# ronen-halevy/yolo-v3-tf2

Hardware: AMD Instinct MI355X
Metric: images/sec at 416x416 batch=64, f32 (full YOLOv3 detect: conv stack + decode + NMS) (higher is better)
Workload: dtype f32

## Files before the change

include/y3.h:

```cpp
#ifndef Y3_H
#define Y3_H

#include <stddef.h>
#include <stdint.h>

#ifdef __cplusplus
extern "C" {
#endif

typedef int y3_status;
enum {
    Y3_OK = 0,
    Y3_ERR_INVALID = -1,
    Y3_ERR_HIP = -2,
    Y3_ERR_OOM = -3,
    Y3_ERR_STATE = -4,
    Y3_ERR_NODEVICE = -5,
    Y3_ERR_COMM = -6,
    Y3_ERR_INTERNAL = -7
};

enum { Y3_DTYPE_F32 = 0, Y3_DTYPE_BF16 = 1, Y3_DTYPE_F32X3 = 2, Y3_DTYPE_F32X2 = 3, Y3_DTYPE_F16 = 4, Y3_DTYPE_I8 = 5 };

int y3_version(void);
// ... 22 lines not shown

enum { Y3_AUX_ADD = 0, Y3_AUX_UPSAMPLE2X = 1, Y3_AUX_CONCAT = 2 };
typedef struct {
    int32_t kind;
    int32_t src0;
    int32_t src1;
    int32_t dst;
} y3_aux_desc;

typedef struct {
    int32_t channels;
    int32_t div;
} y3_tensor_desc;

y3_status y3_net_create(const y3_tensor_desc *tensors, int n_tensors, const int32_t *op_kinds, int n_ops,
                        const y3_conv_desc *convs, int n_convs, const y3_aux_desc *aux, int n_aux,
                        int input_tensor, const int32_t outputs[3], int nclasses, y3_net **out);
void y3_net_destroy(y3_net *net);

y3_status y3_net_set_conv_weights(y3_net *net, int conv_slot, const float *w, const float *gamma,
                                  const float *beta, const float *mean, const float *var, const float *bias,
                                  float eps);

y3_status y3_net_set_tile(y3_net *net, int conv_slot, int tile);
y3_status y3_net_set_tile_bf16(y3_net *net, int conv_slot, int tile);
y3_status y3_net_set_tile_x3(y3_net *net, int conv_slot, int tile);
y3_status y3_net_set_tile_x2(y3_net *net, int conv_slot, int tile);
y3_status y3_net_set_lanes(y3_net *net, int lanes);
y3_status y3_net_set_xcd_mode(y3_net *net, int mode);
y3_status y3_net_set_k_chunk(y3_net *net, int channels);
y3_status y3_net_set_border_skip(y3_net *net, int mode);
int y3_net_get_border_skip(const y3_net *net, int conv_slot, int batch);
void y3_border_order(int Ho, int Wo, int H, int W, int stride, int pad, uint32_t *out);
y3_status y3_net_set_low_latency(y3_net *net, int on);
y3_status y3_net_set_split_k(y3_net *net, int conv_slot, int S);
int y3_net_get_split_k(const y3_net *net, int conv_slot);
int y3_choose_split_k(long long tiles, int k_tiles, int n_cus, long long slab_bytes_per_slice);
y3_status y3_net_set_low_latency_bf16(y3_net *net, int on);
y3_status y3_net_set_split_k_bf16(y3_net *net, int conv_slot, int S);
int y3_net_get_split_k_bf16(const y3_net *net, int conv_slot);
y3_status y3_net_set_low_latency_f16(y3_net *net, int on);
y3_status y3_net_set_split_k_f16(y3_net *net, int conv_slot, int S);
int y3_net_get_split_k_f16(const y3_net *net, int conv_slot);
y3_status y3_net_keep_activations(y3_net *net, int keep);
y3_status y3_net_set_stem_fusion(y3_net *net, int on);
y3_status y3_net_set_stem_fusion_f16(y3_net *net, int on);
y3_status y3_net_measure_sclk(y3_net *net, const float *images_dev, int batch, float *const grids_dev[3], int forwards,
                              float *mhz_out, void *stream);
y3_status y3_net_measure_sclk_conv(y3_net *net, const float *images_dev, int batch, float *const grids_dev[3], int forwards,
                                   int conv, float *mhz_out, void *stream);
y3_status y3_net_measure_sclk_all(y3_net *net, const float *images_dev, int batch, float *const grids_dev[3], int forwards,
                                  float *mhz_out, double *start_us, double *end_us, void *stream);
y3_status y3_net_set_early_chunk(y3_net *net, int n_convs, int chunk_images);

y3_status y3_net_plan(y3_net *net, int max_batch, int image_size, int dtype);

y3_status y3_net_plan_hw(y3_net *net, int max_batch, int height, int width, int dtype);

y3_status y3_net_forward(y3_net *net, const float *images_dev, int batch, float *const grids_dev[3], void *stream);

y3_status y3_net_read_tensor(y3_net *net, int tensor_id, int batch, float *dst_dev, size_t *n_elems, void *stream);

y3_status y3_net_set_act_scales(y3_net *net, const float *scales, int n_tensors);
float y3_net_get_act_scale(const y3_net *net, int tensor_id);
int y3_net_i8_first_conv(const y3_net *net);
y3_status y3_net_read_tensor_i8(y3_net *net, int tensor_id, int batch, int8_t *dst_dev, size_t *n_elems, void *stream);
// ... 89 lines not shown
```

yolo-v3-tf2_amd/_lib.py:

```python
from __future__ import annotations

import ctypes as C
import os

from . import PACKAGE_DIR

LIB_PATH = os.environ.get("Y3_LIB_PATH") or os.path.join(PACKAGE_DIR, "lib", "liby3hip.so")

Y3_OK = 0
Y3_DTYPE_F32, Y3_DTYPE_BF16, Y3_DTYPE_F32X3, Y3_DTYPE_F32X2, Y3_DTYPE_F16, Y3_DTYPE_I8 = 0, 1, 2, 3, 4, 5
DTYPE_TAGS = {Y3_DTYPE_F32: "f32", Y3_DTYPE_BF16: "bf16", Y3_DTYPE_F32X3: "f32x3", Y3_DTYPE_F32X2: "f32x2", Y3_DTYPE_F16: "f16", Y3_DTYPE_I8: "i8"}
TILES_I8_BUILT = (8, 10, 11, 12, 17, 19, 24, 26, 27, 29)
TILES_X2_BUILT = (0, 1, 2, 3, 4, 8, 12, 26, 27)
TILES_X3_BUILT = (0, 1, 2, 3, 4, 8, 9, 12, 13, 14)
Y3_AUX_ADD, Y3_AUX_UPSAMPLE2X, Y3_AUX_CONCAT = 0, 1, 2
_Z = (0, 0, 0, 0)
TILES = [_Z, _Z, _Z, _Z, _Z, _Z,
         (128, 128, 4, 1), _Z, (256, 32, 4, 1), (128, 64, 4, 1), (64, 128, 4, 1), (64, 64, 4, 1),
         (128, 128, 8, 1), _Z, _Z, _Z,
         _Z, (128, 64, 8, 1), _Z, _Z,
         _Z, _Z, _Z,
         (128, 128, 4, 1), _Z,
         _Z,
         (64, 128, 4, 2), (64, 64, 4, 2), _Z, _Z, _Z,
# ... 42 lines not shown
class TensorDesc(C.Structure):
    _fields_ = [("channels", C.c_int32), ("div", C.c_int32)]


class ImageDesc(C.Structure):
    _fields_ = [("offset", C.c_uint64), ("height", C.c_int32), ("width", C.c_int32), ("channels", C.c_int32),
                ("mode", C.c_int32)]


_vp, _i, _f, _sz = C.c_void_p, C.c_int, C.c_float, C.c_size_t
_fp = C.POINTER(C.c_float)

SYMBOLS = {
    "y3_version": (_i, []),
    "y3_last_error": (C.c_char_p, []),
    "y3_device_count": (_i, []),
    "y3_tile_built": (_i, [_i, _i]),
    "y3_net_create": (_i, [C.POINTER(TensorDesc), _i, C.POINTER(C.c_int32), _i, C.POINTER(ConvDesc), _i,
                           C.POINTER(AuxDesc), _i, _i, C.POINTER(C.c_int32), _i, C.POINTER(_vp)]),
    "y3_net_destroy": (None, [_vp]),
    "y3_net_set_conv_weights": (_i, [_vp, _i, _fp, _fp, _fp, _fp, _fp, _fp, _f]),
    "y3_net_set_tile": (_i, [_vp, _i, _i]),
    "y3_net_set_tile_bf16": (_i, [_vp, _i, _i]),
    "y3_net_set_tile_x3": (_i, [_vp, _i, _i]),
    "y3_net_set_tile_x2": (_i, [_vp, _i, _i]),
    "y3_net_set_early_chunk": (_i, [_vp, _i, _i]),
    "y3_net_keep_activations": (_i, [_vp, _i]),
    "y3_net_set_lanes": (_i, [_vp, _i]),
    "y3_net_set_xcd_mode": (_i, [_vp, _i]),
    "y3_net_set_k_chunk": (_i, [_vp, _i]),
    "y3_net_set_border_skip": (_i, [_vp, _i]),
    "y3_net_get_border_skip": (_i, [_vp, _i, _i]),
    "y3_border_order": (None, [_i, _i, _i, _i, _i, _i, C.POINTER(C.c_uint32)]),
    "y3_net_set_stem_fusion": (_i, [_vp, _i]),
    "y3_net_set_low_latency": (_i, [_vp, _i]),
    "y3_net_set_split_k": (_i, [_vp, _i, _i]),
    "y3_net_get_split_k": (_i, [_vp, _i]),
    "y3_choose_split_k": (_i, [C.c_longlong, _i, _i, C.c_longlong]),
    "y3_net_set_low_latency_bf16": (_i, [_vp, _i]),
    "y3_net_set_split_k_bf16": (_i, [_vp, _i, _i]),
    "y3_net_get_split_k_bf16": (_i, [_vp, _i]),
    "y3_net_set_low_latency_f16": (_i, [_vp, _i]),
    "y3_net_set_split_k_f16": (_i, [_vp, _i, _i]),
    "y3_net_get_split_k_f16": (_i, [_vp, _i]),
    "y3_net_set_stem_fusion_f16": (_i, [_vp, _i]),
    "y3_net_measure_sclk": (_i, [_vp, _vp, _i, C.POINTER(_vp), _i, _fp, _vp]),
    "y3_net_measure_sclk_conv": (_i, [_vp, _vp, _i, C.POINTER(_vp), _i, _i, _fp, _vp]),
    "y3_net_measure_sclk_all": (_i, [_vp, _vp, _i, C.POINTER(_vp), _i, _fp, C.POINTER(C.c_double), C.POINTER(C.c_double), _vp]),
    "y3_net_plan": (_i, [_vp, _i, _i, _i]),
    "y3_net_plan_hw": (_i, [_vp, _i, _i, _i, _i]),
    "y3_net_forward": (_i, [_vp, _vp, _i, C.POINTER(_vp), _vp]),
    "y3_net_read_tensor": (_i, [_vp, _i, _i, _vp, C.POINTER(_sz), _vp]),
    "y3_net_set_act_scales": (_i, [_vp, _fp, _i]),
    "y3_net_get_act_scale": (_f, [_vp, _i]),
    "y3_net_i8_first_conv": (_i, [_vp]),
    "y3_net_read_tensor_i8": (_i, [_vp, _i, _i, _vp, C.POINTER(_sz), _vp]),
    "y3_net_flops_per_image": (C.c_double, [_vp]),
    "y3_net_profile_convs": (_i, [_vp, _vp, _i, _fp, _i, _vp]),
    "y3_preprocess_image": (_i, [_vp, _i, _i, _i, _i, _vp, _i, _i, _vp]),
    "y3_preprocess_image_hw": (_i, [_vp, _i, _i, _i, _i, _vp, _i, _i, _i, _vp]),
    "y3_preprocess_batch": (_i, [_vp, _sz, C.POINTER(ImageDesc), _i, _vp, _i, _i, _vp]),
    "y3_preprocess_batch_hw": (_i, [_vp, _sz, C.POINTER(ImageDesc), _i, _vp, _i, _i, _i, _vp]),
    "y3_letterbox_geometry": (_i, [C.POINTER(ImageDesc), _i, _i, C.POINTER(C.c_int32)]),
    "y3_letterbox_geometry_hw": (_i, [C.POINTER(ImageDesc), _i, _i, _i, C.POINTER(C.c_int32)]),
    "y3_unletterbox_detections": (_i, [_vp, _vp, C.POINTER(C.c_int32), _i, _i, _i, _vp]),
    "y3_unletterbox_detections_hw": (_i, [_vp, _vp, C.POINTER(C.c_int32), _i, _i, _i, _i, _vp]),
# ... 74 lines not shown
```

yolo-v3-tf2_amd/csrc/conv_f32.hip:

```cpp
#include <algorithm>
#include <type_traits>

#include "conv_common.h"

namespace y3 {

static constexpr int BK = 32;
static constexpr int lds_row(int dma) { return dma ? BK : BK + 4; }

__device__ __forceinline__ f32x4 buf_load16(__amdgpu_buffer_rsrc_t r, unsigned voff, int soff)
{
    u32x4 v = __builtin_amdgcn_raw_buffer_load_b128(r, (int)voff, soff, 0);
    return __builtin_bit_cast(f32x4, v);
}

#ifdef Y3_PHASE_STAMPS
__device__ unsigned long long y3_dbg32_stamps[8 * 32768];
__device__ int y3_dbg32_sel_k = -1;
#define Y3_STAMP32(k) do { if (threadIdx.x == 0 && blockIdx.x < 32768 && p.K == y3_dbg32_sel_k) y3_dbg32_stamps[blockIdx.x * 8 + (k)] = __builtin_amdgcn_s_memrealtime(); } while (0)
#else
#define Y3_STAMP32(k) do { } while (0)
#endif

template <int TM, int TN, int WR, int WC, bool CONCAT, int STAGES, int MINW = 1, int DMA = 0, bool SPLIT = false, bool BMIN = false>
// ... 12 lines not shown
    constexpr int LDS_ROW = lds_row(DMA);
    constexpr int BM = 32 * TM * WR;
    constexpr int BN = 32 * TN * WC;
    constexpr int NT = 64 * WR * WC;
    constexpr int RP = NT / 8;
    constexpr int AP = BM / RP;
    constexpr int BP = BN / RP;
    static_assert(BM % RP == 0 && BN % RP == 0 && AP >= 1 && BP >= 1, "tile too small for the thread count");
    constexpr int STAGE = (BM + BN) * LDS_ROW;
    extern __shared__ __attribute__((aligned(16))) float smem[];

    const int tid = threadIdx.x;
    if constexpr (!SPLIT) clk_stamp_entry(p.clk_stamps);
    const int lane = tid & 63;
    const int wave = __builtin_amdgcn_readfirstlane(tid >> 6);
    const int wr = wave / WC, wc = wave % WC;

    const int nwg = gridDim.x;
    const int bid = blockIdx.x, xcd = bid & 7;
    const int logical = xcd_contiguous_tile(bid, nwg);
    const int tilesN = p.CoutPad / BN;
    const int kt0 = SPLIT ? (int)blockIdx.y * (p.K / BK) / (int)gridDim.y : 0;
    int KT = SPLIT ? ((int)blockIdx.y + 1) * (p.K / BK) / (int)gridDim.y - kt0 : p.K / BK;
    const __amdgpu_buffer_rsrc_t rs0 = buffer_rsrc(p.src0, p.src0_bytes);
    const __amdgpu_buffer_rsrc_t rs1 = buffer_rsrc(CONCAT ? p.src1 : p.src0, CONCAT ? p.src1_bytes : p.src0_bytes);
    const __amdgpu_buffer_rsrc_t rsw = buffer_rsrc(p.wpk, p.w_bytes);
    const unsigned OOB0 = p.src0_bytes, OOB1 = CONCAT ? p.src1_bytes : p.src0_bytes;

    const __amdgpu_buffer_rsrc_t rsd = buffer_rsrc(p.dst, p.dst_bytes);
    const __amdgpu_buffer_rsrc_t rsr = buffer_rsrc(p.residual ? p.residual : p.dst, p.dst_bytes);
    const int fr = lane & 31, fh = lane >> 5;

    int mt = logical / tilesN, nt = logical - mt * tilesN;
    if (p.xcd_gn > 0) {
        const int gn = p.xcd_gn, gm = 8 / gn;
        const int tilesM = (p.M + BM - 1) / BM;
        const int xm = xcd / gn, xn = xcd - xm * gn;
        const int nb = tilesN / gn;
        const int mlo = xm * tilesM / gm, mhi = (xm + 1) * tilesM / gm;
        const int j = bid >> 3;
        const int lm = j / nb;
        mt = mlo + lm;
        nt = xn * nb + (j - lm * nb);
        if (mt >= mhi) return;
    }
    const int m0 = mt * BM, n0 = nt * BN;

    const int lrow = tid >> 3;
    const int lchunk = DMA ? swizzled_chunk<8>(lrow, tid & 7) * 4 : (tid & 7) * 4;
    int aoff[AP];
    int aoff1[CONCAT ? AP : 1];
    int ahw[AP];
    const int C1 = p.Cin - p.C0;
    constexpr int NBLK = BMIN ? BM / 32 : 1;
    TileBlocks blk{0, 0, 1, 0x1ffu};
    unsigned eent[BMIN ? TM : 1];
    int eimg[BMIN ? TM : 1];
    if constexpr (BMIN) {
        blk = tile_blocks<NBLK>(p, m0);
        if (blk.live == 0) blk.live = 1;
        KT = __builtin_popcount(blk.live) * (p.Cin / BK);
#pragma unroll
        for (int i = 0; i < TM; ++i) tile_block<NBLK>(p, blk, wr * TM + i, eent[i], eimg[i]);
    } else {
        const TileOrigin org = tile_origin(p, m0);
#pragma unroll
        for (int i = 0; i < AP; ++i)
// ... 308 lines not shown
    const int m = (int)(idx / per_row);
    const int n = ((int)(idx - (size_t)m * per_row)) * W;
    const float *src = ws + (size_t)m * cout_pad + n;
    vec v = *reinterpret_cast<const vec *>(src);
    for (int s = 1; s < S; ++s) v = v + *reinterpret_cast<const vec *>(src + (size_t)s * slab_elems);
    v = v + *reinterpret_cast<const vec *>(shift + n);
    if (leaky) {
        const vec t = v * 0.1f;
#pragma unroll
        for (int k = 0; k < W; ++k) v[k] = fmaxf(v[k], t[k]);
    }
    const size_t o = (size_t)m * cout + n;
    if (residual) v = *reinterpret_cast<const vec *>(residual + o) + v;
    *reinterpret_cast<vec *>(dst + o) = v;
}

template <int TM, int TN, int WR, int WC, bool CONCAT, int STAGES, int MINW, int DMA>
static hipError_t launch_k(const ConvArgs &a, hipStream_t s)
{
    constexpr int BM = 32 * TM * WR, BN = 32 * TN * WC;
    const int tilesM = (a.M + BM - 1) / BM, tilesN = a.CoutPad / BN;
    const size_t lds = STAGES * (size_t)(BM + BN) * lds_row(DMA) * sizeof(float);
    int grid = tilesM * tilesN;
    if (a.xcd_gn > 0) {
        if (8 % a.xcd_gn || tilesN % a.xcd_gn) return hipErrorInvalidValue;
        const int gm = 8 / a.xcd_gn;
        int rows = 0;
        for (int xm = 0; xm < gm; ++xm) rows = std::max(rows, (xm + 1) * tilesM / gm - xm * tilesM / gm);
        grid = 8 * rows * (tilesN / a.xcd_gn);
    }
    if constexpr (!CONCAT) {
        if (a.pos_tab) {
            if (a.ksize != 3 || a.B < 32 || a.B % 32 || a.M != a.B * a.Ho * a.Wo || a.Ho > kPosMaxGrid || a.Wo > kPosMaxGrid) return hipErrorInvalidValue;
            return launch_conv_kernel<conv_f32_mfma<TM, TN, WR, WC, false, STAGES, MINW, DMA, false, true>>(a, grid, 64 * WR * WC, lds, s);
        }
    } else if (a.pos_tab) {
        return hipErrorInvalidValue;
    }
    return launch_conv_kernel<conv_f32_mfma<TM, TN, WR, WC, CONCAT, STAGES, MINW, DMA>>(a, grid, 64 * WR * WC, lds, s);
}

template <int TM, int TN, int WR, int WC, int STAGES, int MINW, int DMA>
static hipError_t launch_t(const ConvArgs &a, hipStream_t s)
{
    return a.src1 ? launch_k<TM, TN, WR, WC, true, STAGES, MINW, DMA>(a, s) : launch_k<TM, TN, WR, WC, false, STAGES, MINW, DMA>(a, s);
}

struct TileF32 { TileInfo info; hipError_t (*launch)(const ConvArgs &, hipStream_t); };
template <int TM, int TN, int WR, int WC, int STAGES = 1, int MINW = 1, int DMA = 0>
static constexpr TileF32 tile() { return {{32 * TM * WR, 32 * TN * WC, WR * WC, STAGES, BK}, launch_t<TM, TN, WR, WC, STAGES, MINW, DMA>}; }

static hipError_t launch_res(const ConvArgs &a, hipStream_t s) { return conv_res_f32_fits(a) ? launch_conv_res_f32(a, s) : hipErrorInvalidValue; }

static const TileF32 kTiles[TILE_COUNT] = {
    {}, {}, {}, {}, {}, {},
    tile<2, 2, 2, 2>(),
    {},
    tile<2, 1, 4, 1>(),
    tile<1, 2, 4, 1, 1, 4>(),
    tile<1, 2, 2, 2, 1, 4>(),
    tile<1, 1, 2, 2, 1, 4>(),
    tile<2, 1, 2, 4>(),
    {}, {}, {}, {},
    tile<1, 1, 4, 2>(),
    {}, {}, {}, {}, {},
    tile<2, 2, 2, 2, 1, 3>(),
// ... 57 lines not shown
```

yolo-v3-tf2_amd/csrc/y3_forward.cpp:

```cpp
#include <cstdlib>
#include <vector>

#include "y3_host.h"

struct Forward {
    const float *images;
    float *const *grids;
    int batch;
    hipStream_t stream;
    int lanes;
    const y3::DecodeHead *heads = nullptr;
    unsigned long long *clk = nullptr;
    int clk_conv = -1;
    float *ms_out = nullptr;
    int n_ms = 0;
};

static y3_status check_forward_args(const y3_net *net, bool args_ok, int batch, bool heads, const char *who)
{
    if (!net || !args_ok || batch <= 0) return fail(Y3_ERR_INVALID, "%s: bad argument", who);
    if (heads && net->nclasses <= 0) return fail(Y3_ERR_STATE, "%s: the net was created without detection heads (nclasses = 0)", who);
    if (!net->height) return fail(Y3_ERR_STATE, "%s: call y3_net_plan first", who);
    if (batch > net->max_batch) return fail(Y3_ERR_INVALID, "%s: batch %d > planned %d", who, batch, net->max_batch);
    return Y3_OK;
// ... 159 lines not shown
        if (x.kind == Y3_AUX_ADD)
            e = y3::launch_add(p(x.src0), p(x.src1), p(x.dst), (size_t)nb * sh * sw * C, s);
        else if (x.kind == Y3_AUX_UPSAMPLE2X)
            e = y3::launch_upsample2x(p(x.src0), nb, sh / 2, sw / 2, C, p(x.dst), s);
        else if (x.kind == Y3_AUX_CONCAT)
            e = y3::launch_concat(p(x.src0), net->tensors[x.src0].channels, p(x.src1), net->tensors[x.src1].channels, (size_t)nb * sh * sw, p(x.dst), s);
        else
            return fail(Y3_ERR_INVALID, "unknown aux op kind %d", x.kind);
        if (e != hipSuccess) return fail(Y3_ERR_HIP, "aux op %d launch: %s", index, hipGetErrorString(e));
        return Y3_OK;
    }

    y3_status run(int op_begin, int op_end) const
    {
        hipEvent_t ev0 = nullptr, ev1 = nullptr;
        if (f.ms_out) {
            HIP_TRY(hipEventCreate(&ev0));
            HIP_TRY(hipEventCreate(&ev1));
        }
        if (op_begin == 0 && crosses(net->input_tensor))
            if (y3_status st = quantize_crossing(net->input_tensor); st != Y3_OK) return st;
        for (int oi = op_begin; oi < op_end; ++oi) {
            const Op &o = net->ops[oi];
            if (o.kind != 0) {
                if (y3_status st = run_aux(o.index); st != Y3_OK) return st;
                continue;
            }
            y3::ConvArgs a = conv_args(o.index);
            if (!a.src0 || (!a.dst && !a.dec.boxes)) return fail(Y3_ERR_STATE, "conv %d: tensor not planned", o.index);
            const y3::ConvChoice ch = y3::choose_conv(net, oi, a);
            a.k_chunk = ch.k_chunk;
            a.xcd_gn = ch.xcd_gn;
            a.pos_tab = ch.pos_tab;
            if (ch.kind == y3::ConvKind::InStem) {
                if (f.ms_out && o.index < f.n_ms) f.ms_out[o.index] = 0.0f;
            } else {
                if (f.ms_out) HIP_TRY(hipEventRecord(ev0, s));
                if (y3_status st = launch_conv(oi, a, ch); st != Y3_OK) return st;
                if (f.ms_out) {
                    HIP_TRY(hipEventRecord(ev1, s));
                    HIP_TRY(hipEventSynchronize(ev1));
                    float ms = 0;
                    HIP_TRY(hipEventElapsedTime(&ms, ev0, ev1));
                    if (o.index < f.n_ms) f.ms_out[o.index] = ms;
                }
            }
            const int dst = net->convs[o.index].d.dst;
            if (crosses(dst))
                if (y3_status st = quantize_crossing(dst); st != Y3_OK) return st;
        }
        for (int k = 0; k < 3 && op_end == (int)net->ops.size(); ++k) {
            const int t = net->outputs[k];
            if (!net->staged[t]) continue;
            const size_t npix = (size_t)nb * rows(net, t) * cols(net, t);
            float *out = f.grids[k] + (size_t)b0 * img_elems(t);
            hipError_t e = net->dtype != Y3_DTYPE_I8 ? y3::launch_to_f32(net->dtype, ptr(t), out, npix, net->tensors[t].channels, s)
                           : net->telem[t] == 1      ? y3::launch_i8_to_f32(ptr(t), out, npix * net->tensors[t].channels, net->tscale[t], s)
                                                     : y3::launch_to_f32(Y3_DTYPE_F16, ptr(t), out, npix, net->tensors[t].channels, s);
            if (e != hipSuccess) return fail(Y3_ERR_HIP, "output %d conversion: %s", k, hipGetErrorString(e));
        }
        if (f.ms_out) {
            (void)hipEventDestroy(ev0);
            (void)hipEventDestroy(ev1);
        }
        return Y3_OK;
    }
// ... 320 lines not shown
```

yolo-v3-tf2_amd/csrc/y3_host.h:

```cpp
#pragma once
#include <hip/hip_runtime.h>

#include <vector>

#include "../../include/y3.h"
#include "y3_kernels.h"

namespace y3 {
int fail_msg(int code, const char *fmt, ...) noexcept;
int on_exception(const char *who) noexcept;
bool test_fail_alloc() noexcept;
}

#define Y3_CATCH(who) catch (...) { return y3::on_exception(who); }

constexpr auto fail = y3::fail_msg;

#define HIP_TRY(expr)                                                                             \
    do {                                                                                          \
        hipError_t e_ = (expr);                                                                   \
        if (e_ != hipSuccess)                                                                     \
            return fail(e_ == hipErrorOutOfMemory ? Y3_ERR_OOM : Y3_ERR_HIP, "%s: %s", #expr,     \
                        hipGetErrorString(e_));                                                   \
    } while (0)
// ... 17 lines not shown
struct ConvSlot {
    y3_conv_desc d{};
    bool loaded = false;
    bool first_layer = false;
    int cout_pad = 0;
    int K = 0;
    int tile = -1;
    int split_req = -1;
    int split_req_bf16 = -1;
    int split_req_f16 = -1;
    int split_k = 1;
    int tile_bf16 = -1;
    int tile_x3 = -1;
    int cout_pad64 = 0;
    void *wx3_dev = nullptr;
    int tile_x2 = -1;
    bool x2_ok = true;
    void *wx2_dev = nullptr;
    float *scale_x2_dev = nullptr;
    void *w_dev = nullptr;
    float *w0stem_dev = nullptr;
    float *w0raw_dev = nullptr;
    float *w0norm_dev = nullptr;
    float *scale0norm_dev = nullptr;
    void *wbf_dev = nullptr;
    void *wf16_dev = nullptr;
    float *scale_dev = nullptr;
    float *shift_dev = nullptr;
    void *wi8_dev = nullptr;
    std::vector<float> sw_host, bn_scale_host;
    float *sc_i8_dev = nullptr;
    float q_res = 0.0f, q_inv = 0.0f;
    const uint32_t *pos_tab = nullptr;
};

struct Op {
    int kind;
    int index;
};

constexpr int Y3_MAX_LANES = 4;
constexpr int Y3_MAX_OUTPUT_BOXES = 1024;

struct y3_net {
    int device = 0;
    int n_cus = 0;
    std::vector<y3_tensor_desc> tensors;
    std::vector<Op> ops;
    std::vector<ConvSlot> convs;
    std::vector<y3_aux_desc> aux;
    int input_tensor = 0;
    int outputs[3] = {0, 0, 0};
    int nclasses = 0;
    int max_batch = 0, height = 0, width = 0, dtype = Y3_DTYPE_F32;
    int keep_all = 0;
    int lanes = 1;
    int early_convs = 0;
    int early_chunk = 0;
    int early_ops = 0;
    std::vector<char> dense;
    std::vector<char> staged;
    std::vector<signed char> out_slot;
    void *det_buf = nullptr;
    size_t det_bytes = 0;
    int stem_mode = 1;
    bool stem_mode_set = false;
    int stem_mode_f16 = 0;
    bool stem_fused = false;
    bool stem_conv2 = false;
    int xcd_mode = 1;
    bool low_latency_set = false;
    bool low_latency = false;
    bool low_latency_bf16 = false;
    bool low_latency_f16 = false;
    void *split_ws = nullptr;
    size_t split_ws_lane = 0;
    int split_ws_lanes = 0;
    int k_chunk = -1;
    int border_skip = -1;
    struct PosTab { int Ho, Wo, H, W, stride; uint32_t *dev; };
    std::vector<PosTab> pos_tabs;
    hipEvent_t fork_ev = nullptr;
    hipStream_t lane_stream[4] = {nullptr, nullptr, nullptr, nullptr};
    hipEvent_t join_ev[4] = {nullptr, nullptr, nullptr, nullptr};
    std::vector<void *> tdev;
    std::vector<size_t> tbytes;
    std::vector<size_t> tblock;
    std::vector<void *> blocks;
    std::vector<float> act_scale;
    int i8_first_conv = -1;
    std::vector<unsigned char> telem;
    std::vector<char> tcross;
    std::vector<void *> tq8;
    std::vector<float> tscale;
};

inline int rows(const y3_net *n, int t) { return n->height / n->tensors[t].div; }
inline int cols(const y3_net *n, int t) { return n->width / n->tensors[t].div; }
inline bool is_output(const y3_net *net, int t) { return t == net->outputs[0] || t == net->outputs[1] || t == net->outputs[2]; }

namespace y3 {

struct ConvChoice;
struct SplitForm {
    bool (*tile)(int);
    hipError_t (*launch)(const ConvArgs &, int tile, bool out_f32, int S, void *ws, size_t ws_bytes, hipStream_t);
    int bk, min_k_tiles;
    int ConvSlot::*req;
    bool y3_net::*low_latency;
    const char *set_split, *set_switch;
    const char *(*no_form)(int tile);
    const char *tiles, *other_plan;
    int cout_mult;
// ... 3 lines not shown
    int count;
    TileInfo (*info)(int);
    bool (*built)(int);
    int ConvSlot::*tile;
    int ConvSlot::*cout_pad;
    const char *bad, *retired, *misfit;
    int resident;
    y3_status (*resident_rule)(const y3_net *, const ConvSlot &, int slot);
    void *ConvSlot::*w;
    int elem_bytes;
    int (*choose)(const ConvSlot &, long long M, long long M_plan, bool arena_out);
    hipError_t (*launch)(const ConvArgs &, int tile, bool out_f32, hipStream_t);
    void (*refine)(const y3_net *, const ConvSlot &, const ConvArgs &, ConvChoice &);
    hipError_t (*launch_stem)(const StemArgs &, hipStream_t);
    float *ConvSlot::*w0_stem;
    float *ConvSlot::*scale0_stem;
    int y3_net::*stem_mode;
    const SplitForm *split;
};
const ConvFamily *conv_family(int dtype);
inline const ConvFamily &family_of(const y3_net *net) { return *conv_family(net->dtype); }
inline bool conv_is_i8(const y3_net *net, int slot) { return net->dtype == Y3_DTYPE_I8 && net->i8_first_conv >= 0 && slot >= net->i8_first_conv; }
inline int dtype_of_conv(const y3_net *net, int slot) { return net->dtype != Y3_DTYPE_I8 || conv_is_i8(net, slot) ? net->dtype : (int)Y3_DTYPE_F16; }
inline const ConvFamily &family_of_conv(const y3_net *net, int slot) { return *conv_family(dtype_of_conv(net, slot)); }

enum class ConvKind { First, Stem, InStem, HeadDecodeF32, Mfma, SplitK };
struct ConvChoice {
    ConvKind kind;
    int tile;
    int k_chunk;
    int xcd_gn;
    int split_k;
    const uint32_t *pos_tab;
};
ConvChoice choose_conv(const y3_net *net, int oi, const ConvArgs &a);
ConvChoice choose_conv_planned(const y3_net *net, int oi);
int conv_op(const y3_net *net, int slot);

bool stem_applicable(const y3_net *net);
bool stem_conv2_applicable(const y3_net *net);
void resolve_stem(y3_net *net);
bool output_staged(const y3_net *net, int t);
y3_status resolve_splits(y3_net *net);
y3_status resolve_border(y3_net *net);
y3_status resolve_i8(y3_net *net);
y3_status upload_i8_scales(y3_net *net, int slot);
void free_plan(y3_net *net);

struct DetectLayout {
    int32_t gs[3][2];
    size_t n_boxes;
    size_t grid[3], boxes, cls, scores, sel, nms_ws, total;
};
DetectLayout detect_layout(const y3_net *net, int batch);

y3_status decode_scores_hw(const char *who, const float *const grids_dev[3], const int32_t (*grid_hw)[2], int batch, int nclasses,
                           const float *anchors_host, float *bboxes_dev, int64_t *class_idx_dev, float *scores_dev, void *stream);

}
```

yolo-v3-tf2_amd/csrc/y3_kernels.h:

```cpp
#pragma once
#include <hip/hip_runtime.h>
#include <stddef.h>
#include <stdint.h>
#include <type_traits>

#include "../../include/y3.h"
#include "decode_box.h"

namespace y3 {

struct ConvArgs {
    const void *src0;
    const void *src1;
    const void *wpk;
    const float *scale;
    const float *shift;
    const void *residual;
    void *dst;
    int B, H, W;
    int Ho, Wo;
    int Cin, C0;
    int Cout, CoutPad;
    int ksize, stride, pad;
    int up0;
    int leaky;
    int M;
    int K;
    unsigned src0_bytes, src1_bytes, w_bytes, dst_bytes;
    int xcd_gn;
    DecodeHead dec;
    int k_chunk;
    unsigned long long *clk_stamps;
    int n_cus;
    int device;
    float q_res, q_inv;
    const uint32_t *pos_tab;
};

constexpr int kPosMaxGrid = 2047;
constexpr int kPosTabPad = 8;
constexpr uint32_t pos_pack(int ho, int wo, uint32_t mask9) { return ((uint32_t)ho << 20) | ((uint32_t)wo << 9) | mask9; }
constexpr int pos_ho(uint32_t e) { return (int)(e >> 20); }
constexpr int pos_wo(uint32_t e) { return (int)((e >> 9) & 0x7ffu); }
constexpr uint32_t pos_mask(uint32_t e) { return e & 0x1ffu; }
void border_order(int Ho, int Wo, int H, int W, int stride, int pad, uint32_t *out);

struct LdsAttrOnce { unsigned long long done = 0; };
inline hipError_t set_max_lds_once(LdsAttrOnce &st, const void *fn, int bytes, int dev = -1)
{
    hipError_t e = hipSuccess;
    if (dev < 0 && (e = hipGetDevice(&dev)) != hipSuccess) return e;
    if (dev >= 0 && dev < 64 && ((st.done >> dev) & 1ull)) return hipSuccess;
    e = hipFuncSetAttribute(fn, hipFuncAttributeMaxDynamicSharedMemorySize, bytes);
    if (e == hipSuccess && dev >= 0 && dev < 64) st.done |= 1ull << dev;
    return e;
}

template <auto KERNEL>
static hipError_t launch_conv_kernel(const ConvArgs &a, int grid, int threads, size_t lds, hipStream_t s, int grid_y = 1)
{
    if (lds > 160 * 1024) return hipErrorInvalidValue;
    static LdsAttrOnce attr;
    if (hipError_t e = set_max_lds_once(attr, reinterpret_cast<const void *>(KERNEL), (int)lds, a.device); e != hipSuccess) return e;
    hipLaunchKernelGGL(KERNEL, dim3(grid, grid_y), dim3(threads), lds, s, a);
    return hipGetLastError();
}

template <typename LAUNCH>
static hipError_t dispatch_concat_out(bool concat, bool out_f32, LAUNCH launch)
{
// ... 152 lines not shown
```

yolo-v3-tf2_amd/csrc/y3_net.cpp:

```cpp
#include <algorithm>
#include <cmath>
#include <cstdarg>
#include <cstdio>
#include <cstdlib>
#include <cstring>
#include <exception>
#include <memory>
#include <new>

#include "y3_host.h"

namespace {

thread_local char g_err[512] = "";

}

namespace y3 {
int fail_msg(int code, const char *fmt, ...) noexcept
{
    va_list ap;
    va_start(ap, fmt);
    vsnprintf(g_err, sizeof(g_err), fmt, ap);
    va_end(ap);
// ... 202 lines not shown
        return blocks(27) >= 512 ? 27 : 29;
    }
    if (bf16_out && c.d.size == 3 && c.d.stride == 1 && c.d.src1 < 0 && (c.d.cin == 32 || c.d.cin == 64) && c.d.cout % 64 == 0) return 32;
    static constexpr int bk32[] = {5, 6},
                         n128[] = {8, 12, 11},
                         n64[] = {10, 11}, n32[] = {4};
    if (c.d.cin % 64) return first_reaching(bk32, y3::conv_bf16_tile_info, c, c.cout_pad, M, 512);
    if (c.cout_pad % 128 == 0) return first_reaching(n128, y3::conv_bf16_tile_info, c, c.cout_pad, M, 512);
    if (c.cout_pad % 64 == 0) return first_reaching(n64, y3::conv_bf16_tile_info, c, c.cout_pad, M, 512);
    return first_reaching(n32, y3::conv_bf16_tile_info, c, c.cout_pad, M, 512);
}

int choose_tile_i8(const ConvSlot &c, long long M, long long M_plan, bool arena_out)
{
    const int t = choose_tile_bf16(c, M, M_plan, arena_out);
    if (y3::conv_i8_tile_built(t) && fits(y3::conv_i8_tile_info(t), c, c.cout_pad64)) return t;
    static constexpr int n64[] = {10, 11};
    return first_reaching(n64, y3::conv_i8_tile_info, c, c.cout_pad64, M, 512);
}

int default_k_chunk(const ConvSlot &c)
{
    static const int env = [] { const char *e = getenv("Y3_K_CHUNK"); return e ? atoi(e) : -1; }();
    if (env >= 0) return env;
    return (c.d.size == 3 && c.d.cin >= 256) ? 128 : 0;
}

constexpr int kBorderSkipMaxPositions = 1 << 30;
bool default_border_skip(const y3::ConvArgs &a)
{
    static const int env = [] { const char *e = getenv("Y3_BORDER_SKIP"); return e ? atoi(e) : -1; }();
    static const int max_pos = [] { const char *e = getenv("Y3_BORDER_SKIP_MAX_POS"); return e ? atoi(e) : kBorderSkipMaxPositions; }();
    return env != 0 && a.Ho * a.Wo <= max_pos;
}

int choose_xcd_gn(const ConvSlot &c, const y3::ConvArgs &a, const y3::TileInfo &t)
{
    const int tilesN = a.CoutPad / t.bn;
    const long long tilesM = (a.M + t.bm - 1) / t.bm;
    if (tilesM * tilesN < 64) return 0;
    const double w_bytes = (double)a.CoutPad * c.K * 4.0, a_bytes = (double)a.src0_bytes + a.src1_bytes;
    int best = 0;
    double best_cost = 0;
    for (int gn = 1; gn <= 8; gn *= 2) {
        const int gm = 8 / gn;
        if (tilesN % gn || tilesM < gm) continue;
        double cost = gn * a_bytes + gm * w_bytes;
        if (w_bytes / gn > 2.5e6) cost += 8.0 * (a_bytes + w_bytes);
        if (!best || cost < best_cost) {
            best = gn;
            best_cost = cost;
        }
    }
    return best > 1 ? best : 0;
}

int choose_tile(const ConvSlot &c, long long M, long long, bool)
{
    if (c.d.size == 3 && c.d.stride == 1 && c.d.src1 < 0 && c.d.cin == 32 && c.d.cout % 64 == 0 && c.cout_pad == c.d.cout) return 33;
    static constexpr int n128[] = {10, 11}, n64[] = {11}, n32[] = {8};
    if (c.cout_pad % 128 == 0) return first_reaching(n128, y3::conv_tile_info, c, c.cout_pad, M, 1024);
    if (c.cout_pad % 64 == 0) return first_reaching(n64, y3::conv_tile_info, c, c.cout_pad, M, 1024);
    return first_reaching(n32, y3::conv_tile_info, c, c.cout_pad, M, 1024);
}

}
// ... 46 lines not shown
        if (c.d.dst == t && (c.d.residual >= 0 || c.first_layer)) return true;
    }
    return false;
}

namespace {

y3_status resident_rule_f32(const y3_net *, const ConvSlot &c, int)
{
    if (!(c.d.size == 3 && c.d.stride == 1 && c.d.src1 < 0 && c.d.cin == 32 && c.d.cout % 64 == 0))
        return fail(Y3_ERR_INVALID, "y3_net_set_tile: tile 33 (weight-resident) needs a 3x3 / stride-1 conv with 32 input channels and Cout %% 64 == 0");
    return Y3_OK;
}

y3_status resident_rule_bf16(const y3_net *net, const ConvSlot &c, int slot)
{
    if (!(c.d.size == 3 && c.d.stride == 1 && c.d.src1 < 0 && (c.d.cin == 32 || c.d.cin == 64) && c.d.cout % 64 == 0))
        return fail(Y3_ERR_INVALID, "y3_net_set_tile_bf16: tile 32 (weight-resident) needs a 3x3 / stride-1 conv with 32 or 64 input channels and Cout %% 64 == 0");
    if (is_output(net, c.d.dst) && !y3::output_staged(net, c.d.dst))
        return fail(Y3_ERR_INVALID, "y3_net_set_tile_bf16: tile 32 (weight-resident) stores bf16 only; conv %d writes an fp32 net output", slot);
    return Y3_OK;
}

void refine_f32(const y3_net *net, const ConvSlot &c, const y3::ConvArgs &a, y3::ConvChoice &ch)
{
    if (a.dec.boxes) { ch.kind = y3::ConvKind::HeadDecodeF32; return; }
    ch.split_k = c.split_k;
    if (c.split_k > 1) ch.kind = y3::ConvKind::SplitK;
    else if (net->xcd_mode) ch.xcd_gn = choose_xcd_gn(c, a, y3::conv_tile_info(ch.tile));
    const int ck = net->k_chunk >= 0 ? net->k_chunk : default_k_chunk(c);
    if (c.d.size == 3 && c.d.src1 < 0 && ck > 0 && c.d.cin > ck && c.d.cin % ck == 0 && ck % 32 == 0) ch.k_chunk = ck;
    const bool legal = c.pos_tab && ch.kind == y3::ConvKind::Mfma && ch.tile != 33 && a.B >= 32 && a.B % 32 == 0 &&
                       (long long)a.Ho * a.Wo * a.Cout * 4 * 32 < 0x7fffffffLL;
    if (legal && (net->border_skip >= 0 ? net->border_skip == 1 : default_border_skip(a))) ch.pos_tab = c.pos_tab;
}

void refine_bf16(const y3_net *, const ConvSlot &c, const y3::ConvArgs &a, y3::ConvChoice &ch)
{
    if (c.split_k > 1 && !a.dec.boxes) {
        ch.split_k = c.split_k;
        ch.kind = y3::ConvKind::SplitK;
        return;
    }
    if (a.dec.boxes && y3::conv_bf16_tile_info(ch.tile).bn != 256) {
        const bool m16 = ch.tile >= 24 && ch.tile <= 29;
        const bool big = (a.M + 255) / 256 >= 256;
        ch.tile = m16 ? (big ? 24 : 26) : (big ? 17 : 19);
    }
}

hipError_t launch_f32(const y3::ConvArgs &a, int tile, bool, hipStream_t s) { return y3::launch_conv_f32(a, tile, s); }
hipError_t launch_f32_split(const y3::ConvArgs &a, int tile, bool, int S, void *ws, size_t n, hipStream_t s) { return y3::launch_conv_f32_split(a, tile, S, ws, n, s); }

#ifndef Y3_SPLIT_MIN_K_TILES_BF16
#define Y3_SPLIT_MIN_K_TILES_BF16 32
#endif
constexpr int kSplitMinKTilesBf16 = Y3_SPLIT_MIN_K_TILES_BF16;

constexpr y3::SplitForm F32_SPLIT = {
    y3::conv_split_tile, launch_f32_split, 32, 0, &ConvSlot::split_req, &y3_net::low_latency, "y3_net_set_split_k", "y3_net_set_low_latency",
    [](int) { return "the conv's tile has no split form (tiles 10 and 11 have; the weight-resident tile 33 and the 32-wide tile 8 have not)"; },
    "tiles 10 and 11 have",
    "only Y3_DTYPE_F32 plans split K", 1, nullptr};
constexpr y3::SplitForm BF16_SPLIT = {
    y3::conv_bf16_split_tile, y3::launch_conv_bf16_split, 64, kSplitMinKTilesBf16, &ConvSlot::split_req_bf16, &y3_net::low_latency_bf16,
    "y3_net_set_split_k_bf16", "y3_net_set_low_latency_bf16",
    [](int tile) { return tile == 32 ? "the weight-resident tile 32 has no split form" : y3::conv_bf16_tile_info(tile).bk == 32
// ... 33 lines not shown
    "y3_net_set_tile_x2: bad argument", "y3_net_set_tile_x2: tile does not fit this conv", "y3_net_set_tile_x2: tile does not fit this conv", -1, nullptr,
    &ConvSlot::wx2_dev, 4, choose_tile_x2, y3::launch_conv_f32x2, nullptr, nullptr, nullptr, nullptr, nullptr, nullptr};

constexpr y3::ConvFamily I8_FAMILY = {
    y3::BF16_TILE_COUNT, y3::conv_i8_tile_info, y3::conv_i8_tile_built, &ConvSlot::tile_bf16, &ConvSlot::cout_pad64,
    BF16_FAMILY.bad, BF16_FAMILY.retired, BF16_FAMILY.misfit, -1, nullptr,
    &ConvSlot::wi8_dev, 1, choose_tile_i8, y3::launch_conv_i8, refine_bf16, y3::launch_conv_stem_f16, &ConvSlot::w0norm_dev, &ConvSlot::scale0norm_dev,
    &y3_net::stem_mode_f16, nullptr};

int family_tile(const y3::ConvFamily &f, const ConvSlot &c, long long M, long long M_plan, bool arena_out)
{
    const int t = c.*f.tile;
    return t >= 0 && f.built(t) && fits(f.info(t), c, c.*f.cout_pad) ? t : f.choose(c, M, M_plan, arena_out);
}

}

const y3::ConvFamily *y3::conv_family(int dtype)
{
    switch (dtype) {
        case Y3_DTYPE_F32: return &F32_FAMILY;
        case Y3_DTYPE_BF16: return &BF16_FAMILY;
        case Y3_DTYPE_F32X3: return &X3_FAMILY;
        case Y3_DTYPE_F32X2: return &X2_FAMILY;
        case Y3_DTYPE_F16: return &F16_FAMILY;
        case Y3_DTYPE_I8: return &I8_FAMILY;
        default: return nullptr;
    }
}

y3::ConvChoice y3::choose_conv(const y3_net *net, int oi, const ConvArgs &a)
{
    const ConvSlot &c = net->convs[net->ops[oi].index];
    ConvChoice ch{ConvKind::Mfma, -1, 0, 0, 1};
    if ((net->stem_fused && oi == 0) || (net->stem_conv2 && oi == 2)) ch.kind = ConvKind::InStem;
    else if (net->stem_fused && oi == 1) ch.kind = ConvKind::Stem;
    else if (c.first_layer) ch.kind = ConvKind::First;
    if (ch.kind != ConvKind::Mfma) return ch;
    const ConvFamily &f = family_of_conv(net, net->ops[oi].index);
    ch.tile = family_tile(f, c, a.M, (long long)net->max_batch * a.Ho * a.Wo, net->out_slot[c.d.dst] < 0);
    if (f.refine) f.refine(net, c, a, ch);
    return ch;
}

y3::ConvChoice y3::choose_conv_planned(const y3_net *net, int oi)
{
    const ConvSlot &c = net->convs[net->ops[oi].index];
    ConvArgs a{};
    a.Ho = net->height / c.d.out_div;
    a.Wo = net->width / c.d.out_div;
    a.M = net->max_batch * a.Ho * a.Wo;
    a.CoutPad = c.*family_of_conv(net, net->ops[oi].index).cout_pad;
    return choose_conv(net, oi, a);
}

int y3::conv_op(const y3_net *net, int slot)
{
    for (int oi = 0; oi < (int)net->ops.size(); ++oi)
        if (net->ops[oi].kind == 0 && net->ops[oi].index == slot) return oi;
    return -1;
}

static y3_status set_forced_tile(const y3::ConvFamily &f, y3_net *net, int slot, int tile)
{
    if (!net || slot < 0 || slot >= (int)net->convs.size() || tile >= f.count) return fail(Y3_ERR_INVALID, "%s", f.bad);
    ConvSlot &c = net->convs[slot];
    if (tile >= 0) {
// ... 444 lines not shown
```

yolo-v3-tf2_amd/csrc/y3_plan.cpp:

```cpp
#include <algorithm>
#include <cstdlib>

#include "y3_host.h"

void y3::free_plan(y3_net *n)
{
    if (n->det_buf) (void)hipFree(n->det_buf);
    n->det_buf = nullptr;
    n->det_bytes = 0;
    if (n->split_ws) (void)hipFree(n->split_ws);
    n->split_ws = nullptr;
    n->split_ws_lane = 0;
    n->split_ws_lanes = 0;
    for (const y3_net::PosTab &t : n->pos_tabs) (void)hipFree(t.dev);
    n->pos_tabs.clear();
    for (ConvSlot &c : n->convs) c.pos_tab = nullptr;
    for (void *p : n->blocks) (void)hipFree(p);
    n->blocks.clear();
    n->tdev.assign(n->tensors.size(), nullptr);
    n->tq8.assign(n->tensors.size(), nullptr);
}

void y3::border_order(int Ho, int Wo, int H, int W, int stride, int pad, uint32_t *out)
{
    auto mask_of = [&](int ho, int wo) {
        uint32_t mk = 0;
        for (int u = 0; u < 3; ++u)
            for (int v = 0; v < 3; ++v) {
                const int hi = ho * stride - pad + u, wi = wo * stride - pad + v;
                if (hi >= 0 && hi < H && wi >= 0 && wi < W) mk |= 1u << (u * 3 + v);
            }
        return mk;
    };
    auto key_of = [](uint32_t mk) { return (uint32_t)__builtin_popcount(mk) * 512u + mk; };
    std::vector<int> at(10 * 512 + 1, 0);
    for (int ho = 0; ho < Ho; ++ho)
        for (int wo = 0; wo < Wo; ++wo) ++at[key_of(mask_of(ho, wo)) + 1];
    for (int k = 0; k < 10 * 512; ++k) at[k + 1] += at[k];
    for (int ho = 0; ho < Ho; ++ho)
        for (int wo = 0; wo < Wo; ++wo) {
            const uint32_t mk = mask_of(ho, wo);
            out[at[key_of(mk)]++] = pos_pack(ho, wo, mk);
        }
}

y3_status y3::resolve_border(y3_net *net)
{
    if (net->dtype != Y3_DTYPE_F32) return Y3_OK;
    for (ConvSlot &c : net->convs) {
        const y3_conv_desc &d = c.d;
        if (d.size != 3 || d.src1 >= 0 || c.first_layer) continue;
        const y3_net::PosTab g{net->height / d.out_div, net->width / d.out_div, net->height / d.in_div, net->width / d.in_div, d.stride, nullptr};
        if (g.Ho > kPosMaxGrid || g.Wo > kPosMaxGrid) continue;
        for (const y3_net::PosTab &t : net->pos_tabs)
            if (t.Ho == g.Ho && t.Wo == g.Wo && t.H == g.H && t.W == g.W && t.stride == g.stride) c.pos_tab = t.dev;
        if (c.pos_tab) continue;
        const size_t n = (size_t)g.Ho * g.Wo;
        std::vector<uint32_t> tab(n + kPosTabPad, 0u);
        border_order(g.Ho, g.Wo, g.H, g.W, g.stride, 1, tab.data());
        net->pos_tabs.push_back(g);
        y3_net::PosTab &t = net->pos_tabs.back();
        HIP_TRY(hipMalloc(reinterpret_cast<void **>(&t.dev), tab.size() * sizeof(uint32_t)));
        HIP_TRY(hipMemcpy(t.dev, tab.data(), tab.size() * sizeof(uint32_t), hipMemcpyHostToDevice));
        c.pos_tab = t.dev;
    }
    return Y3_OK;
}

static y3_status ensure_lanes(y3_net *net)
{
    if (net->fork_ev) return Y3_OK;
    HIP_TRY(hipEventCreateWithFlags(&net->fork_ev, hipEventDisableTiming));
    for (int i = 0; i < Y3_MAX_LANES; ++i) {
        HIP_TRY(hipStreamCreateWithFlags(&net->lane_stream[i], hipStreamNonBlocking));
        HIP_TRY(hipEventCreateWithFlags(&net->join_ev[i], hipEventDisableTiming));
    }
    return Y3_OK;
}

static y3_status place_tensors(y3_net *net, const std::vector<int> &first, const std::vector<int> &last)
{
    const int nt = (int)net->tensors.size();
    struct Blk { void *p; size_t bytes; int free_at; };
    std::vector<Blk> pool;
    std::vector<int> order;
    for (int t = 0; t < nt; ++t) {
        const bool external = t == net->input_tensor || net->out_slot[t] >= 0;
        if (first[t] >= 0 && !external) order.push_back(t);
    }
    std::sort(order.begin(), order.end(), [&](int a, int b) { return first[a] < first[b]; });
    for (int t : order) {
        const int until = (net->keep_all || net->dense[t]) ? (int)net->ops.size() + 1 : last[t];
        int pick = -1;
        for (int k = 0; k < (int)pool.size() && !net->dense[t]; ++k)
            if (pool[k].free_at < first[t] && pool[k].bytes >= net->tbytes[t] &&
                (pick < 0 || pool[k].bytes < pool[pick].bytes))
                pick = k;
// ... 200 lines not shown
        if (env >= 0 && env <= 2 && !net->stem_mode_set) net->stem_mode = env;
    }
    y3::resolve_stem(net);
    {
        static const int env = [] { const char *e = getenv("Y3_LOW_LATENCY"); return e ? atoi(e) : -1; }();
        if ((env == 0 || env == 1) && !net->low_latency_set) net->low_latency = env == 1;
    }
    if (net->nclasses > 0) {
        const size_t bytes = y3::detect_layout(net, max_batch).total;
        hipError_t e = hipMalloc(&net->det_buf, bytes);
        if (e != hipSuccess) {
            y3::free_plan(net);
            return fail(Y3_ERR_OOM, "y3_net_plan: hipMalloc(%zu) for the detect scratch failed: %s", bytes, hipGetErrorString(e));
        }
        net->det_bytes = bytes;
    }
    if (y3_status st = y3::resolve_splits(net); st != Y3_OK) {
        y3::free_plan(net);
        return st;
    }
    if (y3_status st = y3::resolve_border(net); st != Y3_OK) {
        y3::free_plan(net);
        return st;
    }
    return Y3_OK;
}
Y3_CATCH("y3_net_plan_hw")

void y3_border_order(int Ho, int Wo, int H, int W, int stride, int pad, uint32_t *out)
{
    if (out && Ho > 0 && Wo > 0 && Ho <= y3::kPosMaxGrid && Wo <= y3::kPosMaxGrid) y3::border_order(Ho, Wo, H, W, stride, pad, out);
}

y3_status y3_net_plan(y3_net *net, int max_batch, int image_size, int dtype)
try {
    return y3_net_plan_hw(net, max_batch, image_size, image_size, dtype);
}
Y3_CATCH("y3_net_plan")

double y3_net_flops_per_image(const y3_net *net)
{
    if (!net || !net->height) return 0.0;
    double tot = 0;
    for (const ConvSlot &c : net->convs) {
        const double ho = net->height / c.d.out_div, wo = net->width / c.d.out_div;
        tot += 2.0 * c.d.size * c.d.size * c.d.cin * c.d.cout * ho * wo;
    }
    return tot;
}

}
```

Before: 2108.

## Balance border and interior M-tiles across XCDs in border-skip conv

Adds a tile-to-workgroup mapping for border-skip 3x3 convs. Each XCD group gets an equal share of the border tiles (which are costlier because of masking) and of the interior tiles, instead of contiguous M ranges that can pile all border tiles onto a few XCDs. The planner records how many positions precede the first full-interior mask and passes a border tile count into the kernel. Grid size is recomputed, and surplus workgroups exit early. The aim is to remove load imbalance across XCDs, at the cost of some index arithmetic and possible idle workgroups. It is on by default and controlled by the Y3_BORDER_BALANCE environment variable.

```diff
diff --git a/include/y3.h b/include/y3.h
--- a/include/y3.h
+++ b/include/y3.h
@@ -78,6 +78,7 @@
 y3_status y3_net_set_border_skip(y3_net *net, int mode);
 int y3_net_get_border_skip(const y3_net *net, int conv_slot, int batch);
 void y3_border_order(int Ho, int Wo, int H, int W, int stride, int pad, uint32_t *out);
+int y3_border_tile_map(int T, int Tb, int gm, int tilesN, int32_t *out);
 y3_status y3_net_set_low_latency(y3_net *net, int on);
 y3_status y3_net_set_split_k(y3_net *net, int conv_slot, int S);
 int y3_net_get_split_k(const y3_net *net, int conv_slot);
diff --git a/yolo-v3-tf2_amd/_lib.py b/yolo-v3-tf2_amd/_lib.py
--- a/yolo-v3-tf2_amd/_lib.py
+++ b/yolo-v3-tf2_amd/_lib.py
@@ -98,6 +98,7 @@
     "y3_net_set_border_skip": (_i, [_vp, _i]),
     "y3_net_get_border_skip": (_i, [_vp, _i, _i]),
     "y3_border_order": (None, [_i, _i, _i, _i, _i, _i, C.POINTER(C.c_uint32)]),
+    "y3_border_tile_map": (_i, [_i, _i, _i, _i, C.POINTER(C.c_int32)]),
     "y3_net_set_stem_fusion": (_i, [_vp, _i]),
     "y3_net_set_low_latency": (_i, [_vp, _i]),
     "y3_net_set_split_k": (_i, [_vp, _i, _i]),
diff --git a/yolo-v3-tf2_amd/csrc/conv_f32.hip b/yolo-v3-tf2_amd/csrc/conv_f32.hip
--- a/yolo-v3-tf2_amd/csrc/conv_f32.hip
+++ b/yolo-v3-tf2_amd/csrc/conv_f32.hip
@@ -68,7 +68,12 @@
     const int fr = lane & 31, fh = lane >> 5;
 
     int mt = logical / tilesN, nt = logical - mt * tilesN;
-    if (p.xcd_gn > 0) {
+    if (BMIN && p.border_tiles >= 0) {
+        const TileMN t = balanced_tile(bid, p.xcd_gn > 0 ? p.xcd_gn : 1, tilesN, p.border_tiles, (p.M + BM - 1) / BM);
+        mt = t.mt;
+        nt = t.nt;
+        if (mt < 0) return;
+    } else if (p.xcd_gn > 0) {
         const int gn = p.xcd_gn, gm = 8 / gn;
         const int tilesM = (p.M + BM - 1) / BM;
         const int xm = xcd / gn, xn = xcd - xm * gn;
@@ -443,6 +448,8 @@
     if constexpr (!CONCAT) {
         if (a.pos_tab) {
             if (a.ksize != 3 || a.B < 32 || a.B % 32 || a.M != a.B * a.Ho * a.Wo || a.Ho > kPosMaxGrid || a.Wo > kPosMaxGrid) return hipErrorInvalidValue;
+            if (a.border_tiles > tilesM) return hipErrorInvalidValue;
+            if (a.border_tiles >= 0) grid = balanced_grid(a.xcd_gn > 0 ? a.xcd_gn : 1, tilesN, a.border_tiles, tilesM);
             return launch_conv_kernel<conv_f32_mfma<TM, TN, WR, WC, false, STAGES, MINW, DMA, false, true>>(a, grid, 64 * WR * WC, lds, s);
         }
     } else if (a.pos_tab) {
diff --git a/yolo-v3-tf2_amd/csrc/y3_forward.cpp b/yolo-v3-tf2_amd/csrc/y3_forward.cpp
--- a/yolo-v3-tf2_amd/csrc/y3_forward.cpp
+++ b/yolo-v3-tf2_amd/csrc/y3_forward.cpp
@@ -215,6 +215,7 @@
             a.k_chunk = ch.k_chunk;
             a.xcd_gn = ch.xcd_gn;
             a.pos_tab = ch.pos_tab;
+            a.border_tiles = ch.border_tiles;
             if (ch.kind == y3::ConvKind::InStem) {
                 if (f.ms_out && o.index < f.n_ms) f.ms_out[o.index] = 0.0f;
             } else {
diff --git a/yolo-v3-tf2_amd/csrc/y3_host.h b/yolo-v3-tf2_amd/csrc/y3_host.h
--- a/yolo-v3-tf2_amd/csrc/y3_host.h
+++ b/yolo-v3-tf2_amd/csrc/y3_host.h
@@ -73,6 +73,7 @@
     float *sc_i8_dev = nullptr;
     float q_res = 0.0f, q_inv = 0.0f;
     const uint32_t *pos_tab = nullptr;
+    int pos_border = 0;
 };
 
 struct Op {
@@ -119,7 +120,7 @@
     int split_ws_lanes = 0;
     int k_chunk = -1;
     int border_skip = -1;
-    struct PosTab { int Ho, Wo, H, W, stride; uint32_t *dev; };
+    struct PosTab { int Ho, Wo, H, W, stride; uint32_t *dev; int border; };
     std::vector<PosTab> pos_tabs;
     hipEvent_t fork_ev = nullptr;
     hipStream_t lane_stream[4] = {nullptr, nullptr, nullptr, nullptr};
@@ -189,6 +190,7 @@
     int xcd_gn;
     int split_k;
     const uint32_t *pos_tab;
+    int border_tiles;
 };
 ConvChoice choose_conv(const y3_net *net, int oi, const ConvArgs &a);
 ConvChoice choose_conv_planned(const y3_net *net, int oi);
diff --git a/yolo-v3-tf2_amd/csrc/y3_kernels.h b/yolo-v3-tf2_amd/csrc/y3_kernels.h
--- a/yolo-v3-tf2_amd/csrc/y3_kernels.h
+++ b/yolo-v3-tf2_amd/csrc/y3_kernels.h
@@ -35,7 +35,38 @@
     int device;
     float q_res, q_inv;
     const uint32_t *pos_tab;
+    int border_tiles;
 };
+
+__host__ __device__ inline int balanced_range(int xm, int gm, int Tb, int T)
+{
+    return ((xm + 1) * Tb / gm - xm * Tb / gm) + ((xm + 1) * (T - Tb) / gm - xm * (T - Tb) / gm);
+}
+__host__ __device__ inline int balanced_mtile(int lm, int xm, int gm, int Tb, int T)
+{
+    const int blo = xm * Tb / gm, nb = (xm + 1) * Tb / gm - blo;
+    const int ilo = Tb + xm * (T - Tb) / gm, ni = Tb + (xm + 1) * (T - Tb) / gm - ilo;
+    if (lm >= nb + ni) return -1;
+#ifdef Y3_BORDER_FIRST
+    return lm < nb ? blo + lm : ilo + (lm - nb);
+#else
+    return lm < ni ? ilo + lm : blo + (lm - ni);
+#endif
+}
+struct TileMN { int mt, nt; };
+__host__ __device__ inline TileMN balanced_tile(int bid, int gn, int tilesN, int Tb, int T)
+{
+    const int gm = 8 / gn, xcd = bid & 7, xm = xcd / gn, xn = xcd - xm * gn;
+    const int nb = tilesN / gn, j = bid >> 3, lm = j / nb;
+    return {balanced_mtile(lm, xm, gm, Tb, T), xn * nb + (j - lm * nb)};
+}
+inline int balanced_grid(int gn, int tilesN, int Tb, int T)
+{
+    const int gm = 8 / gn;
+    int rows = 0;
+    for (int xm = 0; xm < gm; ++xm) rows = rows > balanced_range(xm, gm, Tb, T) ? rows : balanced_range(xm, gm, Tb, T);
+    return 8 * rows * (tilesN / gn);
+}
 
 constexpr int kPosMaxGrid = 2047;
 constexpr int kPosTabPad = 8;
diff --git a/yolo-v3-tf2_amd/csrc/y3_net.cpp b/yolo-v3-tf2_amd/csrc/y3_net.cpp
--- a/yolo-v3-tf2_amd/csrc/y3_net.cpp
+++ b/yolo-v3-tf2_amd/csrc/y3_net.cpp
@@ -258,6 +258,11 @@
     static const int env = [] { const char *e = getenv("Y3_BORDER_SKIP"); return e ? atoi(e) : -1; }();
     static const int max_pos = [] { const char *e = getenv("Y3_BORDER_SKIP_MAX_POS"); return e ? atoi(e) : kBorderSkipMaxPositions; }();
     return env != 0 && a.Ho * a.Wo <= max_pos;
+}
+bool border_balance()
+{
+    static const int env = [] { const char *e = getenv("Y3_BORDER_BALANCE"); return e ? atoi(e) : 1; }();
+    return env != 0;
 }
 
 int choose_xcd_gn(const ConvSlot &c, const y3::ConvArgs &a, const y3::TileInfo &t)
@@ -370,7 +375,11 @@
     if (c.d.size == 3 && c.d.src1 < 0 && ck > 0 && c.d.cin > ck && c.d.cin % ck == 0 && ck % 32 == 0) ch.k_chunk = ck;
     const bool legal = c.pos_tab && ch.kind == y3::ConvKind::Mfma && ch.tile != 33 && a.B >= 32 && a.B % 32 == 0 &&
                        (long long)a.Ho * a.Wo * a.Cout * 4 * 32 < 0x7fffffffLL;
-    if (legal && (net->border_skip >= 0 ? net->border_skip == 1 : default_border_skip(a))) ch.pos_tab = c.pos_tab;
+    if (legal && (net->border_skip >= 0 ? net->border_skip == 1 : default_border_skip(a))) {
+        ch.pos_tab = c.pos_tab;
+        const long long bm = y3::conv_tile_info(ch.tile).bm;
+        if (border_balance()) ch.border_tiles = (int)std::min(((long long)c.pos_border * a.B + bm - 1) / bm, (a.M + bm - 1) / bm);
+    }
 }
 
 void refine_bf16(const y3_net *, const ConvSlot &c, const y3::ConvArgs &a, y3::ConvChoice &ch)
@@ -470,7 +479,7 @@
 y3::ConvChoice y3::choose_conv(const y3_net *net, int oi, const ConvArgs &a)
 {
     const ConvSlot &c = net->convs[net->ops[oi].index];
-    ConvChoice ch{ConvKind::Mfma, -1, 0, 0, 1};
+    ConvChoice ch{ConvKind::Mfma, -1, 0, 0, 1, nullptr, -1};
     if ((net->stem_fused && oi == 0) || (net->stem_conv2 && oi == 2)) ch.kind = ConvKind::InStem;
     else if (net->stem_fused && oi == 1) ch.kind = ConvKind::Stem;
     else if (c.first_layer) ch.kind = ConvKind::First;
diff --git a/yolo-v3-tf2_amd/csrc/y3_plan.cpp b/yolo-v3-tf2_amd/csrc/y3_plan.cpp
--- a/yolo-v3-tf2_amd/csrc/y3_plan.cpp
+++ b/yolo-v3-tf2_amd/csrc/y3_plan.cpp
@@ -14,7 +14,10 @@
     n->split_ws_lanes = 0;
     for (const y3_net::PosTab &t : n->pos_tabs) (void)hipFree(t.dev);
     n->pos_tabs.clear();
-    for (ConvSlot &c : n->convs) c.pos_tab = nullptr;
+    for (ConvSlot &c : n->convs) {
+        c.pos_tab = nullptr;
+        c.pos_border = 0;
+    }
     for (void *p : n->blocks) (void)hipFree(p);
     n->blocks.clear();
     n->tdev.assign(n->tensors.size(), nullptr);
@@ -50,19 +53,24 @@
     for (ConvSlot &c : net->convs) {
         const y3_conv_desc &d = c.d;
         if (d.size != 3 || d.src1 >= 0 || c.first_layer) continue;
-        const y3_net::PosTab g{net->height / d.out_div, net->width / d.out_div, net->height / d.in_div, net->width / d.in_div, d.stride, nullptr};
+        const y3_net::PosTab g{net->height / d.out_div, net->width / d.out_div, net->height / d.in_div, net->width / d.in_div, d.stride, nullptr, 0};
         if (g.Ho > kPosMaxGrid || g.Wo > kPosMaxGrid) continue;
         for (const y3_net::PosTab &t : net->pos_tabs)
-            if (t.Ho == g.Ho && t.Wo == g.Wo && t.H == g.H && t.W == g.W && t.stride == g.stride) c.pos_tab = t.dev;
+            if (t.Ho == g.Ho && t.Wo == g.Wo && t.H == g.H && t.W == g.W && t.stride == g.stride) {
+                c.pos_tab = t.dev;
+                c.pos_border = t.border;
+            }
         if (c.pos_tab) continue;
         const size_t n = (size_t)g.Ho * g.Wo;
         std::vector<uint32_t> tab(n + kPosTabPad, 0u);
         border_order(g.Ho, g.Wo, g.H, g.W, g.stride, 1, tab.data());
         net->pos_tabs.push_back(g);
         y3_net::PosTab &t = net->pos_tabs.back();
+        while ((size_t)t.border < n && pos_mask(tab[t.border]) != 0x1ffu) ++t.border;
         HIP_TRY(hipMalloc(reinterpret_cast<void **>(&t.dev), tab.size() * sizeof(uint32_t)));
         HIP_TRY(hipMemcpy(t.dev, tab.data(), tab.size() * sizeof(uint32_t), hipMemcpyHostToDevice));
         c.pos_tab = t.dev;
+        c.pos_border = t.border;
     }
     return Y3_OK;
 }
@@ -329,6 +337,18 @@
     if (out && Ho > 0 && Wo > 0 && Ho <= y3::kPosMaxGrid && Wo <= y3::kPosMaxGrid) y3::border_order(Ho, Wo, H, W, stride, pad, out);
 }
 
+int y3_border_tile_map(int T, int Tb, int gm, int tilesN, int32_t *out)
+{
+    if (T < 1 || Tb < 0 || Tb > T || (gm != 1 && gm != 2 && gm != 4 && gm != 8) || tilesN < 1 || tilesN % (8 / gm)) return -1;
+    const int gn = 8 / gm, grid = y3::balanced_grid(gn, tilesN, Tb, T);
+    for (int bid = 0; out && bid < grid; ++bid) {
+        const y3::TileMN t = y3::balanced_tile(bid, gn, tilesN, Tb, T);
+        out[2 * bid] = t.mt;
+        out[2 * bid + 1] = t.mt < 0 ? -1 : t.nt;
+    }
+    return grid;
+}
+
 y3_status y3_net_plan(y3_net *net, int max_batch, int image_size, int dtype)
 try {
     return y3_net_plan_hw(net, max_batch, image_size, image_size, dtype);
```

After: 2138, median of 6. 1.4% higher.
